# JanisGeise/sparseSpatialSampling

Measured on AMD Instinct MI355X. Metric: Mcells*snapshots/s interpolated, higher is better.
Workload: dtype f64

## Files before the change

### sparsespatialsampling_amd/csrc/interp_plan.hip

```cpp
#include "common.h"
#include "plan_build.h"
#include "point_slots.h"

#include <algorithm>
#include <exception>
#include <memory>
#include <type_traits>
#include <utility>
#include <vector>

struct s3_interp_plan : s3::PlanTables {
    int64_t nc = 0, n_src = 0;
    int k = 0, ucap = 0, tc = 64;
    s3::DevBuf<double> wp;
    bool has_weights = false;
    s3::DevBuf<double> dump;
    size_t dump_doubles = 0;
    s3::DevBuf<int32_t> rows_src;
    int64_t n_table = 0;
    s3::DevBuf<int32_t> sched_begin;
    s3::DevBuf<int32_t> sched_tiles;
    s3::DevBuf<int4> sched_desc;
    s3::DevBuf<double> wl;
    s3::DevBuf<uint16_t> pl;
// ... 195 lines not shown
    const int64_t tile = xcd_block(b, tiles_per_xcd);
    if (tile >= n_tiles) return;
    const int c_begin = tile_cell_begin[tile], n_c = tile_cell_begin[tile + 1] - c_begin;
    const int r_begin = tile_row_begin[tile], n_r = tile_row_begin[tile + 1] - r_begin;
    const bool even_rows = (row_len & 1) == 0;

    const int n_items = n_r * vc;
    V reg[UN];
#pragma unroll
    for (int u = 0; u < UN; ++u) {
        const int item = min(u * BLOCK + (int)threadIdx.x, n_items - 1);
        const int r = item / vc, v = item - r * vc;
        reg[u] = *reinterpret_cast<const V *>(data + (int64_t)rows[r_begin + r] * in_stride + (int64_t)v * EPV);
    }
    const int cl = min((int)threadIdx.x / vc, n_c - 1), v = (int)threadIdx.x - ((int)threadIdx.x / vc) * vc;
    const bool has_item = (int)threadIdx.x < n_c * vc;
    const double *wt = w + (int64_t)c_begin * k + cl;
    const uint16_t *lt = loc + (int64_t)c_begin * k + cl;
    double wr[KMAX];
    int pr[KMAX];
#pragma unroll
    for (int m = 0; m < KMAX; ++m) {
        const int mm = m < k ? m : 0;
        wr[m] = wt[(int64_t)mm * n_c];
        pr[m] = lt[(int64_t)mm * n_c];
    }
    const int64_t cell = perm[c_begin + cl];
#pragma unroll
    for (int u = 0; u < UN; ++u) {
        const int item = u * BLOCK + (int)threadIdx.x;
        if (item < n_items) s_data[item] = reg[u];
    }
    __syncthreads();
    if (!has_item) return;
    double acc[EPV];
#pragma unroll
    for (int i = 0; i < EPV; ++i) acc[i] = 0.0;
#pragma unroll
    for (int m = 0; m < KMAX; ++m) {
        if (m < k) {
            const V a = s_data[pr[m] * vc + v];
            const T *ae = reinterpret_cast<const T *>(&a);
#pragma unroll
            for (int i = 0; i < EPV; ++i) acc[i] = fma(wr[m], (double)ae[i], acc[i]);
        }
    }
    const int64_t col = (int64_t)v * EPV;
    store_piece<EPV>(out + cell * row_len + col, acc, row_len - col, even_rows);
}

template <int J>
__device__ __forceinline__ int quad_bcast_i32(int v) {
    return __builtin_amdgcn_update_dpp(0, v, J | (J << 2) | (J << 4) | (J << 6), 0xf, 0xf, true);
}
template <int J>
__device__ __forceinline__ double quad_bcast_f64(double x) {
    const long long b = __double_as_longlong(x);
    const int lo = quad_bcast_i32<J>((int)(b & 0xffffffffll)), hi = quad_bcast_i32<J>((int)(b >> 32));
    return __longlong_as_double(((long long)hi << 32) | (unsigned int)lo);
}

template <typename T, int KQ>
__global__ void __launch_bounds__(256, 5)
interp_planned_short_quad_kernel(const int32_t *__restrict__ perm, const int32_t *__restrict__ tile_cell_begin,
                                 const int32_t *__restrict__ tile_row_begin, const int32_t *__restrict__ rows,
                                 const uint16_t *__restrict__ loc, const double *__restrict__ w , int k,
                                 const T *__restrict__ data, int64_t row_len, int64_t in_stride, double *__restrict__ out,
                                 int64_t n_tiles, int64_t tiles_per_xcd) {
    using V = typename Vec16<T>::type;
    constexpr int EPV = Vec16<T>::N;
    constexpr int BLOCK = 256, UN = 8, VC = 4;
    extern __shared__ float4 lds_raw[];
    V *s_data = reinterpret_cast<V *>(lds_raw);

    const int64_t b = blockIdx.x;
    const int64_t tile = xcd_block(b, tiles_per_xcd);
    if (tile >= n_tiles) return;
    const int c_begin = tile_cell_begin[tile], n_c = tile_cell_begin[tile + 1] - c_begin;
    const int r_begin = tile_row_begin[tile], n_r = tile_row_begin[tile + 1] - r_begin;
    const bool even_rows = (row_len & 1) == 0;

    const int n_items = n_r * VC;
    V reg[UN];
#pragma unroll
    for (int u = 0; u < UN; ++u) {
        const int item = min(u * BLOCK + (int)threadIdx.x, n_items - 1);
        reg[u] = *reinterpret_cast<const V *>(data + (int64_t)rows[r_begin + (item >> 2)] * in_stride + (int64_t)(item & 3) * EPV);
    }
    const int cl = min((int)threadIdx.x >> 2, n_c - 1), v = (int)threadIdx.x & 3;
    const bool has_item = ((int)threadIdx.x >> 2) < n_c;
    const double *wt = w + (int64_t)c_begin * k + cl;
    const uint16_t *lt = loc + (int64_t)c_begin * k + cl;
    double wq[KQ];
    int pq[KQ];
#pragma unroll
    for (int i = 0; i < KQ; ++i) {
        const int m = i * 4 + v, mm = m < k ? m : 0;
        wq[i] = wt[(int64_t)mm * n_c];
        pq[i] = lt[(int64_t)mm * n_c];
    }
    const int64_t cell = perm[c_begin + cl];
#pragma unroll
    for (int u = 0; u < UN; ++u) {
        const int item = u * BLOCK + (int)threadIdx.x;
        if (item < n_items) s_data[item] = reg[u];
    }
    __syncthreads();
    double acc[EPV];
#pragma unroll
    for (int i = 0; i < EPV; ++i) acc[i] = 0.0;
    auto step = [&](double wm, int pos) {
        const V a = s_data[pos * VC + v];
        const T *ae = reinterpret_cast<const T *>(&a);
#pragma unroll
        for (int i = 0; i < EPV; ++i) acc[i] = fma(wm, (double)ae[i], acc[i]);
    };
#pragma unroll
    for (int i = 0; i < KQ; ++i) {
        const double w0 = quad_bcast_f64<0>(wq[i]), w1 = quad_bcast_f64<1>(wq[i]), w2 = quad_bcast_f64<2>(wq[i]), w3 = quad_bcast_f64<3>(wq[i]);
        const int p0 = quad_bcast_i32<0>(pq[i]), p1 = quad_bcast_i32<1>(pq[i]), p2 = quad_bcast_i32<2>(pq[i]), p3 = quad_bcast_i32<3>(pq[i]);
        if (i * 4 + 0 < k) step(w0, p0);
        if (i * 4 + 1 < k) step(w1, p1);
        if (i * 4 + 2 < k) step(w2, p2);
        if (i * 4 + 3 < k) step(w3, p3);
    }
    if (!has_item) return;
    const int64_t col = (int64_t)v * EPV;
    store_piece<EPV>(out + cell * row_len + col, acc, row_len - col, even_rows);
}

__device__ __forceinline__ void run_map(int64_t b, int64_t tiles_per_xcd, int64_t &tile, int &run) {
    const int64_t i = b >> 3;
    run = (int)(i / tiles_per_xcd);
    tile = (b & 7) * tiles_per_xcd + (i - (int64_t)run * tiles_per_xcd);
}

__device__ __forceinline__ void tail_map(int64_t b, int64_t tiles_per_xcd, int tail, int tail_split, int n_chunks, int64_t &tile,
                                         int &chunk0, int &chunk1) {
    const int64_t i = b >> 3, head = tiles_per_xcd - tail;
    if (i < head) {
        tile = (b & 7) * tiles_per_xcd + i;
        chunk0 = 0;
        chunk1 = n_chunks;
        return;
    }
    const int64_t j = i - head;
    const int run = (int)(j / tail);
    const int per = (n_chunks + tail_split - 1) / tail_split;
    tile = (b & 7) * tiles_per_xcd + head + (j - (int64_t)run * tail);
    chunk0 = run * per;
    chunk1 = chunk0 + per < n_chunks ? chunk0 + per : n_chunks;
}

template <typename T, int TC>
__global__ void __launch_bounds__(TC * 4, 2)
interp_planned_kernel(const int32_t *__restrict__ perm, const int32_t *__restrict__ tile_cell_begin,
                      const int32_t *__restrict__ tile_row_begin, const int32_t *__restrict__ rows,
                      const uint16_t *__restrict__ loc, const double *__restrict__ w , int k, int ucap,
                      const T *__restrict__ data, int64_t row_len, int64_t in_stride, double *__restrict__ out,
                      int64_t n_tiles, int64_t tiles_per_xcd, int chunks_per_block, int n_chunks, int tail, int tail_split) {
    using V = typename Vec16<T>::type;
    constexpr int EPV = Vec16<T>::N;
    constexpr int EPC = PL_SEG / (int)sizeof(T);
    constexpr int BLOCK = TC * 4;
    constexpr int RPP = BLOCK / 8;
    extern __shared__ float4 lds_raw[];
    V *s_data = reinterpret_cast<V *>(lds_raw);
    double *s_w = reinterpret_cast<double *>(lds_raw + (size_t)ucap * 8);
    uint16_t *s_loc = reinterpret_cast<uint16_t *>(s_w + (size_t)k * TC);

    int64_t tile;
    int run = 0, chunk0, chunk1;
    if (tail > 0) {
        tail_map(blockIdx.x, tiles_per_xcd, tail, tail_split, n_chunks, tile, chunk0, chunk1);
    } else {
        run_map(blockIdx.x, tiles_per_xcd, tile, run);
        chunk0 = run * chunks_per_block;
        chunk1 = min(n_chunks, chunk0 + chunks_per_block);
    }
    if (tile >= n_tiles) return;
    chunk0 = __builtin_amdgcn_readfirstlane(chunk0);
    chunk1 = __builtin_amdgcn_readfirstlane(chunk1);
    const int c_begin = tile_cell_begin[tile], n_c = tile_cell_begin[tile + 1] - c_begin;
    const int r_begin = tile_row_begin[tile], n_r = tile_row_begin[tile + 1] - r_begin;
    const bool even_rows = (row_len & 1) == 0;

    stage_tile_tables(w + (int64_t)c_begin * k, loc + (int64_t)c_begin * k, n_c * k, s_w, s_loc, BLOCK);

    const int cl = threadIdx.x >> 2, v0 = threadIdx.x & 3;
    const bool has_cell = cl < n_c;
    const int64_t cell = has_cell ? perm[c_begin + cl] : 0;


    const int srow = threadIdx.x >> 3, svec = threadIdx.x & 7;
#define S3_REP16(X) X(0) X(1) X(2) X(3) X(4) X(5) X(6) X(7) X(8) X(9) X(10) X(11) X(12) X(13) X(14) X(15)
    static_assert(PL_NP == 16, "S3_REP16 expands PL_NP staging passes");
#define S3_DECL(P) const int64_t rbase##P = (int64_t)rows[r_begin + min(P * RPP + srow, n_r - 1)] * in_stride; V preA##P, preB##P;
    S3_REP16(S3_DECL)
#define S3_LOAD_A(P) preA##P = *reinterpret_cast<const V *>(seg_ + rbase##P);
#define S3_LOAD_B(P) preB##P = *reinterpret_cast<const V *>(seg_ + rbase##P);
#define S3_ISSUE(SET, CH)                                            \
    do {                                                             \
        const int64_t c0_ = (int64_t)(CH) * EPC;                     \
        const bool ok_ = c0_ + (int64_t)svec * EPV < row_len;        \
        const T *seg_ = data + c0_ + (ok_ ? svec : 0) * EPV;         \
        S3_REP16(S3_LOAD_##SET)                                      \
    } while (0)
#define S3_STORE_A(P) if (P * RPP + srow < n_r) s_data[(P * RPP + srow) * 8 + svec] = preA##P;
#define S3_STORE_B(P) if (P * RPP + srow < n_r) s_data[(P * RPP + srow) * 8 + svec] = preB##P;

    auto accumulate = [&](int chunk) {
        if (!has_cell) return;
        const int64_t col0 = (int64_t)chunk * EPC;
        double acc0[EPV], acc1[EPV];
#pragma unroll
        for (int i = 0; i < EPV; ++i) acc0[i] = acc1[i] = 0.0;
#pragma unroll 4
        for (int m = 0; m < k; ++m) {
            const int pos = s_loc[m * n_c + cl];
            const double wm = s_w[m * n_c + cl];
            const V a = s_data[pos * 8 + v0];
            const V c = s_data[pos * 8 + v0 + 4];
            const T *ae = reinterpret_cast<const T *>(&a);
            const T *ce = reinterpret_cast<const T *>(&c);
#pragma unroll
            for (int i = 0; i < EPV; ++i) {
                acc0[i] = fma(wm, (double)ae[i], acc0[i]);
                acc1[i] = fma(wm, (double)ce[i], acc1[i]);
            }
        }
        double *o = out + cell * row_len + col0;
        store_piece<EPV>(o + v0 * EPV, acc0, row_len - col0 - (int64_t)v0 * EPV, even_rows);
        store_piece<EPV>(o + (v0 + 4) * EPV, acc1, row_len - col0 - (int64_t)(v0 + 4) * EPV, even_rows);
    };

    if (chunk0 < chunk1) S3_ISSUE(A, chunk0);
    if (chunk0 + 1 < chunk1) S3_ISSUE(B, chunk0 + 1);
    for (int chunk = chunk0; chunk < chunk1; chunk += 2) {
        S3_REP16(S3_STORE_A)
        __syncthreads();
        if (chunk + 2 < chunk1) S3_ISSUE(A, chunk + 2);
        accumulate(chunk);
        __syncthreads();
        if (chunk + 1 >= chunk1) break;
        S3_REP16(S3_STORE_B)
        __syncthreads();
        if (chunk + 3 < chunk1) S3_ISSUE(B, chunk + 3);
        accumulate(chunk + 1);
        __syncthreads();
    }
}

#undef S3_ISSUE
#undef S3_LOAD_A
#undef S3_LOAD_B
#undef S3_STORE_A
#undef S3_STORE_B
#undef S3_DECL

__device__ __forceinline__ float4 select16(bool c, const float4 &a, const float4 &b) {
    return make_float4(c ? a.x : b.x, c ? a.y : b.y, c ? a.z : b.z, c ? a.w : b.w);
}
__device__ __forceinline__ double2 select16(bool c, const double2 &a, const double2 &b) {
    return make_double2(c ? a.x : b.x, c ? a.y : b.y);
}
template <typename T>
__global__ void __launch_bounds__(256, 2)
interp_planned_shift_kernel(const int32_t *__restrict__ perm, const int32_t *__restrict__ tile_cell_begin,
                            const int32_t *__restrict__ tile_row_begin, const int32_t *__restrict__ rows,
                            const uint16_t *__restrict__ loc, const double *__restrict__ w , int k, int ucap,
                            const T *__restrict__ data, int64_t row_len, int64_t in_stride, double *__restrict__ out,
                            int64_t n_tiles, int64_t tiles_per_xcd, int chunks_per_block, int n_chunks, int tail, int tail_split) {
    using V = typename Vec16<T>::type;
    constexpr int TC = 64;
    constexpr int EPV = Vec16<T>::N;
    constexpr int EPC = PL_SEG / (int)sizeof(T);
    constexpr int BLOCK = TC * 4;
    constexpr int RPP = BLOCK / 8;
    extern __shared__ float4 lds_raw[];
    V *s_data = reinterpret_cast<V *>(lds_raw);
    double *s_w = reinterpret_cast<double *>(lds_raw + (size_t)ucap * 8);
    uint16_t *s_loc = reinterpret_cast<uint16_t *>(s_w + (size_t)k * TC);

    int64_t tile;
    int run = 0, chunk0, chunk1;
    if (tail > 0) {
        tail_map(blockIdx.x, tiles_per_xcd, tail, tail_split, n_chunks, tile, chunk0, chunk1);
    } else {
        run_map(blockIdx.x, tiles_per_xcd, tile, run);
        chunk0 = run * chunks_per_block;
        chunk1 = min(n_chunks, chunk0 + chunks_per_block);
    }
    if (tile >= n_tiles) return;
    chunk0 = __builtin_amdgcn_readfirstlane(chunk0);
    chunk1 = __builtin_amdgcn_readfirstlane(chunk1);
    const int c_begin = tile_cell_begin[tile], n_c = tile_cell_begin[tile + 1] - c_begin;
    const int r_begin = tile_row_begin[tile], n_r = tile_row_begin[tile + 1] - r_begin;
    const bool even_rows = (row_len & 1) == 0;

    stage_tile_tables_strided<TC>(w + (int64_t)c_begin * k, loc + (int64_t)c_begin * k, n_c, k, s_w, s_loc);

    const int cl = threadIdx.x >> 2, v0 = threadIdx.x & 3;
    const bool has_cell = cl < n_c;
    const int64_t cell = has_cell ? perm[c_begin + cl] : 0;

    auto accumulate = [&](int chunk) {
        if (!has_cell) return;
        const int64_t col0 = (int64_t)chunk * EPC;
        double acc0[EPV], acc1[EPV];
#pragma unroll
        for (int i = 0; i < EPV; ++i) acc0[i] = acc1[i] = 0.0;
#pragma unroll 4
        for (int m = 0; m < k; ++m) {
            const int pos = s_loc[m * TC + cl];
            const double wm = s_w[m * TC + cl];
            const V a = s_data[pos * 8 + v0];
            const V c = s_data[pos * 8 + v0 + 4];
            const T *ae = reinterpret_cast<const T *>(&a);
            const T *ce = reinterpret_cast<const T *>(&c);
#pragma unroll
            for (int i = 0; i < EPV; ++i) {
                acc0[i] = fma(wm, (double)ae[i], acc0[i]);
                acc1[i] = fma(wm, (double)ce[i], acc1[i]);
            }
        }
        double *o = out + cell * row_len + col0;
        store_piece<EPV>(o + v0 * EPV, acc0, row_len - col0 - (int64_t)v0 * EPV, even_rows);
        store_piece<EPV>(o + (v0 + 4) * EPV, acc1, row_len - col0 - (int64_t)(v0 + 4) * EPV, even_rows);
    };

    const int srow = threadIdx.x >> 3, svec = threadIdx.x & 7;
    const uintptr_t base = reinterpret_cast<uintptr_t>(data);
    const uint64_t stride_bytes = (uint64_t)in_stride * sizeof(T);
    const int n_vec_row = (int)((row_len + EPV - 1) / EPV);
    const int last_vec = n_vec_row - 1;
    const uintptr_t base128 = base & ~(uintptr_t)127;
    char *const lds_raw_bytes = reinterpret_cast<char *>(lds_raw);
    const char *const data128 = reinterpret_cast<const char *>(data) - (base & 127);
    const int j_safe = n_vec_row / 8 - 1;
#define S3H_DECL(P)                                                                                              \
    const char *ptr##P;   \
    uint32_t lds##P;                                  \
    bool old##P;                \
    V preA##P, preB##P;                                                                                          \
    {                                                                                                            \
        const uintptr_t a_ = base + (uint64_t)(uint32_t)rows[r_begin + min(P * RPP + srow, n_r - 1)] * stride_bytes; \
        const int ph_ = (int)(a_ >> 4) & 7;                                                                      \
        ptr##P = data128 + (((a_ & ~(uintptr_t)127) - base128) + 16u * (unsigned)svec) + (int64_t)chunk0 * 128;   \
        old##P = svec >= ph_;                                                                                    \
          \
        lds##P = (uint32_t)(min(P * RPP + srow, n_r - 1) * 8 + ((svec - ph_) & 7)) * 16u;                         \
    }
    S3_REP16(S3H_DECL)
#define S3H_LOAD_FAST(SET, P) pre##SET##P = *reinterpret_cast<const V *>(ptr##P + off_);
#define S3H_LOAD_SAFE(SET, P)                                                                                    \
    {                                                                                                            \
        const int s_ = (int)(lds##P >> 4) & 7;                                             \
        const int d_ = s_ <= svec ? s_ : s_ - 8;                                                   \
        const int over_ = max(0, (J_) * 8 + d_ - last_vec);                                                      \
        pre##SET##P = *reinterpret_cast<const V *>(ptr##P + off_ - 16 * (int64_t)over_);                         \
    }
#define S3H_LOAD_FAST_A(P) S3H_LOAD_FAST(A, P)
#define S3H_LOAD_FAST_B(P) S3H_LOAD_FAST(B, P)
#define S3H_LOAD_SAFE_A(P) S3H_LOAD_SAFE(A, P)
#define S3H_LOAD_SAFE_B(P) S3H_LOAD_SAFE(B, P)
#define S3H_ISSUE(SET, J, AHEAD)                                 \
    do {                                                         \
        constexpr int off_ = (AHEAD) * 128;                      \
        const int J_ = (J);                                      \
        if (J_ <= j_safe) {                                      \
            S3_REP16(S3H_LOAD_FAST_##SET)                        \
        } else {                                                 \
            S3_REP16(S3H_LOAD_SAFE_##SET)                        \
        }                                                        \
    } while (0)
#define S3H_ADVANCE(P) ptr##P += 256;
#define S3H_STORE2(P, OLD, NEW) *reinterpret_cast<V *>(lds_raw_bytes + lds##P) = select16(old##P, OLD, NEW);
#define S3H_STORE_AB(P) S3H_STORE2(P, preA##P, preB##P)
#define S3H_STORE_BA(P) S3H_STORE2(P, preB##P, preA##P)


    if (chunk0 < chunk1) {
        S3H_ISSUE(A, chunk0, 0);
        S3H_ISSUE(B, chunk0 + 1, 1);
    }
    for (int chunk = chunk0; chunk < chunk1; chunk += 2) {
        S3_REP16(S3H_STORE_AB)
        __syncthreads();
        if (chunk + 1 < chunk1) S3H_ISSUE(A, chunk + 2, 2);
        accumulate(chunk);
        __syncthreads();
        if (chunk + 1 >= chunk1) break;
        S3_REP16(S3H_STORE_BA)
        __syncthreads();
        if (chunk + 2 < chunk1) S3H_ISSUE(B, chunk + 3, 3);
        accumulate(chunk + 1);
        __syncthreads();
        S3_REP16(S3H_ADVANCE)
    }
#undef S3H_ADVANCE
#undef S3H_DECL
#undef S3H_LOAD_FAST
#undef S3H_LOAD_SAFE
#undef S3H_LOAD_FAST_A
#undef S3H_LOAD_FAST_B
#undef S3H_LOAD_SAFE_A
#undef S3H_LOAD_SAFE_B
#undef S3H_ISSUE
#undef S3H_STORE2
#undef S3H_STORE_AB
#undef S3H_STORE_BA
}

struct StreamLayoutAligned   { static constexpr int CHUNK_VECS = 8, LP = PL_LP, VOFF = 0, LPR = 8, NPASS = 16; };
struct StreamLayoutUnaligned { static constexpr int CHUNK_VECS = 7, LP = 9, VOFF = 1, LPR = 8, NPASS = 16; };
struct StreamLayoutNarrow    { static constexpr int CHUNK_VECS = 4, LP = 4, VOFF = 0, LPR = 4, NPASS = 8; };

template <int M, int K, bool BOTH, typename T, typename LAY>
__device__ __forceinline__ void stream_read_pair(const int (&pq)[(K + 3) / 4], const typename Vec16<T>::type *__restrict__ s_data,
                                                 int v0, typename Vec16<T>::type (&buf)[4]) {
    if constexpr (M < K) {
        const int pos = quad_bcast_i32<M % 4>(pq[M / 4]);
        buf[0] = s_data[pos * LAY::LP + LAY::VOFF + v0];
        if constexpr (BOTH) buf[1] = s_data[pos * LAY::LP + LAY::VOFF + v0 + 4];
    }
    if constexpr (M + 1 < K) {
        const int pos = quad_bcast_i32<(M + 1) % 4>(pq[(M + 1) / 4]);
        buf[2] = s_data[pos * LAY::LP + LAY::VOFF + v0];
        if constexpr (BOTH) buf[3] = s_data[pos * LAY::LP + LAY::VOFF + v0 + 4];
    }
}

__device__ __forceinline__ double cvt_f64_asm(float x) {
    double d;
    asm volatile("v_cvt_f64_f32_e32 %0, %1" : "=v"(d) : "v"(x));
    return d;
}
__device__ __forceinline__ void fmac_f64_asm(double &acc, double wm, double x) {
    asm volatile("v_fmac_f64_e32 %0, %1, %2" : "+v"(acc) : "v"(wm), "v"(x));
}
template <bool BOTH>
__device__ __forceinline__ void stream_fma_row(double wm, const float4 &a, const float4 &b, double (&acc0)[4], double (&acc1)[4]) {
    if constexpr (BOTH) {
        double t0 = cvt_f64_asm(a.x), t1 = cvt_f64_asm(b.x), t2 = cvt_f64_asm(a.y), t3 = cvt_f64_asm(b.y);
        fmac_f64_asm(acc0[0], wm, t0); t0 = cvt_f64_asm(a.z);
        fmac_f64_asm(acc1[0], wm, t1); t1 = cvt_f64_asm(b.z);
        fmac_f64_asm(acc0[1], wm, t2); t2 = cvt_f64_asm(a.w);
        fmac_f64_asm(acc1[1], wm, t3); t3 = cvt_f64_asm(b.w);
        fmac_f64_asm(acc0[2], wm, t0);
        fmac_f64_asm(acc1[2], wm, t1);
        fmac_f64_asm(acc0[3], wm, t2);
        fmac_f64_asm(acc1[3], wm, t3);
    } else {
        const double t0 = cvt_f64_asm(a.x), t1 = cvt_f64_asm(a.y), t2 = cvt_f64_asm(a.z), t3 = cvt_f64_asm(a.w);
        fmac_f64_asm(acc0[0], wm, t0);
        fmac_f64_asm(acc0[1], wm, t1);
        fmac_f64_asm(acc0[2], wm, t2);
        fmac_f64_asm(acc0[3], wm, t3);
    }
}
template <bool BOTH>
__device__ __forceinline__ void stream_fma_row(double wm, const double2 &a, const double2 &b, double (&acc0)[2], double (&acc1)[2]) {
    acc0[0] = fma(wm, a.x, acc0[0]);
    acc0[1] = fma(wm, a.y, acc0[1]);
    if constexpr (BOTH) {
        acc1[0] = fma(wm, b.x, acc1[0]);
        acc1[1] = fma(wm, b.y, acc1[1]);
    }
}

template <int M, int K, bool BOTH, typename T, typename LAY, typename ISSUE>
__device__ __forceinline__ void stream_accumulate(const double (&wq)[(K + 3) / 4], const int (&pq)[(K + 3) / 4],
                                                  const typename Vec16<T>::type *__restrict__ s_data, int v0,
                                                  typename Vec16<T>::type (&cur)[4], typename Vec16<T>::type (&nxt)[4],
                                                  double (&acc0)[Vec16<T>::N], double (&acc1)[Vec16<T>::N], ISSUE &issue) {
    if constexpr (M < K) {
        stream_read_pair<M + 2, K, BOTH, T, LAY>(pq, s_data, v0, nxt);
        issue(std::integral_constant<int, M / 2>{});
        __builtin_amdgcn_sched_barrier(0);
        stream_fma_row<BOTH>(quad_bcast_f64<M % 4>(wq[M / 4]), cur[0], cur[1], acc0, acc1);
        if constexpr (M + 1 < K) stream_fma_row<BOTH>(quad_bcast_f64<(M + 1) % 4>(wq[(M + 1) / 4]), cur[2], cur[3], acc0, acc1);
        __builtin_amdgcn_sched_barrier(0);
        stream_accumulate<M + 2, K, BOTH, T, LAY>(wq, pq, s_data, v0, nxt, cur, acc0, acc1, issue);
    }
}

template <typename T, int K, bool ALIGNED, bool EVEN, bool NARROW = false>
__global__ void __launch_bounds__(256, 2)
interp_planned_stream_kernel(const int32_t *__restrict__ perm, const int32_t *__restrict__ rows,
                             const uint16_t *__restrict__ pl, const double *__restrict__ wl ,
                             const T *__restrict__ data, int64_t row_len, int64_t in_stride, double *__restrict__ out,
                             double *__restrict__ dump, const int32_t *__restrict__ sched_begin,
                             const int4 *__restrict__ sched_desc, int n_chunks) {
    using V = typename Vec16<T>::type;
    static_assert(!NARROW || ALIGNED, "the narrow layout takes rows on 16-byte boundaries");
    using LAY = std::conditional_t<NARROW, StreamLayoutNarrow, std::conditional_t<ALIGNED, StreamLayoutAligned, StreamLayoutUnaligned>>;
    constexpr int EPV = Vec16<T>::N;
    constexpr int EPC = LAY::CHUNK_VECS * EPV;
    constexpr int BLOCK = 256, RPP = BLOCK / LAY::LPR, NPASS = LAY::NPASS;
    constexpr int KQ = (K + 3) / 4, k = K;
    extern __shared__ float4 lds_raw[];
    V *s_data = reinterpret_cast<V *>(lds_raw);
    int32_t *s_ids = reinterpret_cast<int32_t *>(lds_raw + (size_t)NPASS * RPP * LAY::LP);

    const int tid = threadIdx.x;
    const int my_begin = sched_begin[blockIdx.x], n_my = sched_begin[blockIdx.x + 1] - my_begin;
    if (n_my <= 0) return;
    const int4 *const my_desc = sched_desc + my_begin;
    int lane_zero;
    asm volatile("v_mov_b32 %0, 0" : "=v"(lane_zero));
    auto desc_at = [&](int j) { return my_desc[min(j, n_my - 1) + lane_zero]; };
    const int srow = tid / LAY::LPR, svec = tid % LAY::LPR;
    const int qcl = tid >> 2, v0 = tid & 3;
    double *const dump_lane = dump + ((int64_t)blockIdx.x * BLOCK + tid) * 2;
    const uint32_t stride32 = (uint32_t)in_stride;

#define S3S_DECL(P) int rid##P = 0; V pre##P;
    S3_REP16(S3S_DECL)
    static_assert(PL_NP == 16, "S3_REP16 expands PL_NP staging passes");
    int ida = 0, idb = 0;
    double wq[KQ], wqn[KQ];
    int pq[KQ];
    uint4 pqn_raw;
    int64_t cell = 0;
    int celln = 0;
    int nc_c = 0, nc_n = 0, nr_n = 0;

    auto load_ids = [&](int rb, int nr) {
        ida = rows[rb + min(tid, nr - 1)];
        idb = rows[rb + min(BLOCK + tid, nr - 1)];
    };
    constexpr int NV = (KQ + 1) / 2;
    typedef double wpair_t __attribute__((ext_vector_type(2)));
    auto load_tables = [&](int cb, int nc) {
        nc_n = nc;
        const int cl = min(qcl, nc_n - 1), lane4 = cl * 4 + v0, lanes = nc_n * 4;
        const wpair_t *wv = reinterpret_cast<const wpair_t *>(wl + (int64_t)cb * (4 * NV * 2)) + lane4;
#pragma unroll
        for (int j = 0; j < NV; ++j) {
            const wpair_t two = wv[j * lanes];
            wqn[2 * j] = two.x;
            if (2 * j + 1 < KQ) wqn[2 * j + 1] = two.y;
        }
        pqn_raw = reinterpret_cast<const uint4 *>(pl + (int64_t)cb * 32)[lane4];
        celln = perm[cb + cl];
    };
#define S3S_RID(P) if constexpr (P < NPASS) rid##P = s_ids[min(P * RPP + srow, nr_n - 1)];
#define S3S_LOAD(P)                                                                                                          \
    if constexpr (P < NPASS) {                                                                                               \
        int r_ = rid##P;                                                                                                     \
        asm volatile("" : "+v"(r_));                                           \
        const T *a_ = data + (uint64_t)(uint32_t)r_ * stride32 + c0_;                                                        \
        if constexpr (ALIGNED) {                                                                                             \
            pre##P = *reinterpret_cast<const V *>(a_ + (ok_ ? svec : 0) * EPV);                                              \
        } else {                                                                                                             \
                     \
            const int mis_ = (int)(reinterpret_cast<uintptr_t>(a_) & 15);                                                    \
            const int off_ = 16 * svec - mis_;                                                                               \
            pre##P = *reinterpret_cast<const V *>(reinterpret_cast<const char *>(a_) + (off_ < (int)valid_bytes_ ? off_ : -mis_)); \
        }                                                                                                                    \
    }
#define S3S_LOAD_IF(P) if constexpr (P < NPASS && (P * NS) / NPASS == S) { S3S_LOAD(P) }
#define S3S_ISSUE(CH)                                                                    \
    do {                                                                                 \
        const int64_t c0_ = (int64_t)(CH) * EPC;                                         \
        const bool ok_ = c0_ + (int64_t)svec * EPV < row_len;                            \
        const uintptr_t valid_bytes_ = (uintptr_t)min((int64_t)EPC, row_len - c0_) * sizeof(T);   \
        (void)ok_; (void)valid_bytes_;                                                   \
        S3_REP16(S3S_LOAD)                                                               \
    } while (0)
#define S3S_STORE(P)                                                                                                         \
    if constexpr (P < NPASS) {                                                                                               \
        if constexpr (ALIGNED) {                                                                                             \
            s_data[(P * RPP + srow) * LAY::LP + svec] = pre##P;                                                              \
        } else {                                                                                                             \
            const T *a_ = data + (uint64_t)(uint32_t)rid##P * stride32 + store_c0_;                                          \
            const int ph_ = (int)((reinterpret_cast<uintptr_t>(a_) >> 2) & 3);                                               \
            uint32_t *row_ = reinterpret_cast<uint32_t *>(s_data) + (P * RPP + srow) * (LAY::LP * 4) + 4 + 4 * svec - ph_;   \
            const uint32_t *w_ = reinterpret_cast<const uint32_t *>(&pre##P);                                                \
            row_[0] = w_[0]; row_[1] = w_[1]; row_[2] = w_[2]; row_[3] = w_[3];                                              \
        }                                                                                                                    \
    }

    int4 d_next;
    int2 d_after;
    {
        const int4 d0 = desc_at(0);
        d_next = desc_at(1);
        const int4 d2 = desc_at(2);
        d_after = make_int2(d2.x, d2.y);
        load_ids(d0.x, d0.y);
        s_ids[tid] = ida;
        s_ids[BLOCK + tid] = idb;
        nr_n = d0.y;
        __syncthreads();
        S3_REP16(S3S_RID)
        __syncthreads();
        load_tables(d0.z, d0.w);
        if (n_my > 1) load_ids(d_next.x, d_next.y);
        S3S_ISSUE(0);
    }
    __builtin_amdgcn_sched_barrier(0);
#pragma unroll
    for (int i = 0; i < 8; ++i) *reinterpret_cast<volatile double *>(dump_lane) = 0.0;

    for (int j = 0; j < n_my; ++j) {
#pragma unroll
        for (int i = 0; i < KQ; ++i) {
            wq[i] = wqn[i];
            const uint32_t two = i < 2 ? pqn_raw.x : i < 4 ? pqn_raw.y : i < 6 ? pqn_raw.z : pqn_raw.w;
            pq[i] = (int)((i & 1) ? two >> 16 : two & 0xffffu);
        }
        cell = celln;
        nc_c = nc_n;
        const bool live = qcl < nc_c;
        for (int c = 0; c < n_chunks; ++c) {
            const bool last_chunk = c + 1 == n_chunks;
            const bool enter_next = last_chunk && j + 1 < n_my;
            const int64_t store_c0_ = (int64_t)c * EPC;
            (void)store_c0_;
            S3_REP16(S3S_STORE)
            if (enter_next) {
                s_ids[tid] = ida;
                s_ids[BLOCK + tid] = idb;
            }
            __syncthreads();
            if (enter_next) {
                nr_n = d_next.y;
                S3_REP16(S3S_RID)
                load_tables(d_next.z, d_next.w);
                if (j + 2 < n_my) load_ids(d_after.x, d_after.y);
                d_next = desc_at(j + 2);
                const int4 d3 = desc_at(j + 3);
                d_after = make_int2(d3.x, d3.y);
            }
            const int64_t c0_ = (int64_t)(last_chunk ? 0 : c + 1) * EPC;
            const bool ok_ = c0_ + (int64_t)svec * EPV < row_len;
            const uintptr_t valid_bytes_ = (uintptr_t)min((int64_t)EPC, row_len - c0_) * sizeof(T);
            (void)ok_; (void)valid_bytes_;
            auto issue = [&](auto slot) __attribute__((always_inline)) {
                constexpr int S = decltype(slot)::value, NS = sizeof(T) == 4 ? (K + 1) / 2 : 1;
                S3_REP16(S3S_LOAD_IF)
            };
            const int64_t col0 = (int64_t)c * EPC;
            double acc0[EPV], acc1[EPV];
#pragma unroll
            for (int i = 0; i < EPV; ++i) acc0[i] = acc1[i] = 0.0;
            V buf_a[4], buf_b[4];
            bool upper = false;
            if constexpr (LAY::CHUNK_VECS > 4) upper = col0 + 4 * EPV < row_len;
            if (upper) {
                if constexpr (LAY::CHUNK_VECS > 4) {
                    stream_read_pair<0, K, true, T, LAY>(pq, s_data, v0, buf_a);
                    stream_accumulate<0, K, true, T, LAY>(wq, pq, s_data, v0, buf_a, buf_b, acc0, acc1, issue);
                }
            } else {
                stream_read_pair<0, K, false, T, LAY>(pq, s_data, v0, buf_a);
                stream_accumulate<0, K, false, T, LAY>(wq, pq, s_data, v0, buf_a, buf_b, acc0, acc1, issue);
            }
            __builtin_amdgcn_sched_barrier(0);
            double *const orow = out + cell * row_len;
            const int64_t e0 = col0 + (int64_t)v0 * EPV, e1 = col0 + (int64_t)(v0 + 4) * EPV;
            const bool second = v0 + 4 < LAY::CHUNK_VECS;
            typedef double pair_t __attribute__((ext_vector_type(2), aligned(8)));
#pragma unroll
            for (int i = 0; i < EPV; i += 2) {
                double *p0 = live && e0 + i + 1 < row_len ? orow + e0 + i : dump_lane;
                pair_t v = {acc0[i], acc0[i + 1]};
                *reinterpret_cast<pair_t *>(p0) = v;
            }
            if constexpr (LAY::CHUNK_VECS > 4) {
#pragma unroll
                for (int i = 0; i < EPV; i += 2) {
                    double *p1 = live && second && e1 + i + 1 < row_len ? orow + e1 + i : dump_lane;
                    pair_t v = {acc1[i], acc1[i + 1]};
                    *reinterpret_cast<pair_t *>(p1) = v;
                }
            }
            if constexpr (!EVEN) {
                const int64_t t = row_len - 1;
                double tv = acc0[0];
                bool mine = t == e0;
#pragma unroll
                for (int i = 2; i < EPV; i += 2) {
                    tv = t == e0 + i ? acc0[i] : tv;
                    mine = mine || t == e0 + i;
                }
#pragma unroll
                for (int i = 0; i < EPV; i += 2) {
                    tv = second && t == e1 + i ? acc1[i] : tv;
                    mine = mine || (second && t == e1 + i);
                }
                double *pt = live && mine ? orow + t : dump_lane;
                *pt = tv;
            }
            __syncthreads();
        }
    }
#undef S3S_DECL
#undef S3S_RID
#undef S3S_LOAD
#undef S3S_ISSUE
// ... 604 lines not shown
```

Measured before the change: 124,600.

## Add steady-state rolled prefetch loop with unguarded vector stores in interpolation kernel

Adds a steady-state path for chunks far enough from the row end. Each thread writes its staged vector to LDS and immediately issues the next global load, with scheduling barriers that keep the load ordering fixed. That path skips the fast/safe branch in the issue macro and uses unguarded double2 stores instead of bounds-checked store_piece. Out-of-range threads are clamped to the last cell rather than returning early, so every lane runs uniform code. The aim is to cut branch and bounds overhead and get better load/compute overlap. The risk is that padded lanes now do redundant writes to a valid cell, and the sched barriers can limit compiler scheduling.

Result: faster. 130,100 (median of 6 runs) (+4.4%).

```diff
diff --git a/sparsespatialsampling_amd/csrc/interp_plan.hip b/sparsespatialsampling_amd/csrc/interp_plan.hip
--- a/sparsespatialsampling_amd/csrc/interp_plan.hip
+++ b/sparsespatialsampling_amd/csrc/interp_plan.hip
@@ -521,18 +521,22 @@
 
     const int cl = threadIdx.x >> 2, v0 = threadIdx.x & 3;
     const bool has_cell = cl < n_c;
-    const int64_t cell = has_cell ? perm[c_begin + cl] : 0;
-
-    auto accumulate = [&](int chunk) {
-        if (!has_cell) return;
+    const int64_t cell = perm[c_begin + min(cl, n_c - 1)];
+
+    const int cl_c = min(cl, n_c - 1);
+    auto accumulate = [&](int chunk, auto steady) {
+        constexpr bool STEADY = decltype(steady)::value;
+        if constexpr (!STEADY) {
+            if (!has_cell) return;
+        }
         const int64_t col0 = (int64_t)chunk * EPC;
         double acc0[EPV], acc1[EPV];
 #pragma unroll
         for (int i = 0; i < EPV; ++i) acc0[i] = acc1[i] = 0.0;
 #pragma unroll 4
         for (int m = 0; m < k; ++m) {
-            const int pos = s_loc[m * TC + cl];
-            const double wm = s_w[m * TC + cl];
+            const int pos = s_loc[m * TC + cl_c];
+            const double wm = s_w[m * TC + cl_c];
             const V a = s_data[pos * 8 + v0];
             const V c = s_data[pos * 8 + v0 + 4];
             const T *ae = reinterpret_cast<const T *>(&a);
@@ -544,8 +548,16 @@
             }
         }
         double *o = out + cell * row_len + col0;
-        store_piece<EPV>(o + v0 * EPV, acc0, row_len - col0 - (int64_t)v0 * EPV, even_rows);
-        store_piece<EPV>(o + (v0 + 4) * EPV, acc1, row_len - col0 - (int64_t)(v0 + 4) * EPV, even_rows);
+        if constexpr (STEADY) {
+            double *const ol = o + v0 * EPV;
+#pragma unroll
+            for (int i = 0; i < EPV; i += 2) *reinterpret_cast<double2 *>(ol + i) = make_double2(acc0[i], acc0[i + 1]);
+#pragma unroll
+            for (int i = 0; i < EPV; i += 2) *reinterpret_cast<double2 *>(ol + 4 * EPV + i) = make_double2(acc1[i], acc1[i + 1]);
+        } else {
+            store_piece<EPV>(o + v0 * EPV, acc0, row_len - col0 - (int64_t)v0 * EPV, even_rows);
+            store_piece<EPV>(o + (v0 + 4) * EPV, acc1, row_len - col0 - (int64_t)(v0 + 4) * EPV, even_rows);
+        }
     };
 
     const int srow = threadIdx.x >> 3, svec = threadIdx.x & 7;
@@ -599,24 +611,53 @@
 #define S3H_STORE_BA(P) S3H_STORE2(P, preB##P, preA##P)
 
 
+#define S3H_ROLL_AB(P)                                              \
+    S3H_STORE_AB(P)                                                 \
+    preA##P = *reinterpret_cast<const V *>(ptr##P + 256);           \
+    __builtin_amdgcn_sched_barrier(0);
+#define S3H_ROLL_BA(P)                                              \
+    S3H_STORE_BA(P)                                                 \
+    preB##P = *reinterpret_cast<const V *>(ptr##P + 384);           \
+    ptr##P += 256;                                                  \
+    __builtin_amdgcn_sched_barrier(0);
+#define S3H_STEADY_PAIR(C)                                          \
+    do {                                                            \
+        S3_REP16(S3H_ROLL_AB)                                       \
+        __syncthreads();                                            \
+        accumulate((C), std::true_type());                          \
+        __syncthreads();                                            \
+        S3_REP16(S3H_ROLL_BA)                                       \
+        __syncthreads();                                            \
+        accumulate((C) + 1, std::true_type());                      \
+        __syncthreads();                                            \
+    } while (0)
     if (chunk0 < chunk1) {
         S3H_ISSUE(A, chunk0, 0);
         S3H_ISSUE(B, chunk0 + 1, 1);
     }
-    for (int chunk = chunk0; chunk < chunk1; chunk += 2) {
+    int chunk = chunk0;
+    const int roll_end = min(j_safe, chunk1) - 3;
+    if (even_rows && chunk <= roll_end) {
+        S3H_STEADY_PAIR(chunk);
+        for (chunk += 2; chunk <= roll_end; chunk += 2) S3H_STEADY_PAIR(chunk);
+    }
+    for (; chunk < chunk1; chunk += 2) {
         S3_REP16(S3H_STORE_AB)
         __syncthreads();
         if (chunk + 1 < chunk1) S3H_ISSUE(A, chunk + 2, 2);
-        accumulate(chunk);
+        accumulate(chunk, std::false_type());
         __syncthreads();
         if (chunk + 1 >= chunk1) break;
         S3_REP16(S3H_STORE_BA)
         __syncthreads();
         if (chunk + 2 < chunk1) S3H_ISSUE(B, chunk + 3, 3);
-        accumulate(chunk + 1);
+        accumulate(chunk + 1, std::false_type());
         __syncthreads();
         S3_REP16(S3H_ADVANCE)
     }
+#undef S3H_STEADY_PAIR
+#undef S3H_ROLL_AB
+#undef S3H_ROLL_BA
 #undef S3H_ADVANCE
 #undef S3H_DECL
 #undef S3H_LOAD_FAST
```
